# willard-yuan/cvt

Measured on AMD Instinct MI355X. Metric: queries/sec, OPQ-ADC top-100 over 128-d SIFT-1M, higher is better.
Workload: dtype u8 codes / f32 distances

## Files before the change

### cvt_amd/csrc/adc_mfma.hip

```cpp
#include <algorithm>
#include <cfloat>
#include <cmath>

#include "common.h"
#include "flat_f32_common.h"
#include "adc_scan16.h"
#include "kernels.h"
#include "launch.h"

namespace cvtmi {

namespace {

constexpr double MF_UP = 1.0 + 1e-9;
constexpr double MF_BMAX = 4194304.0;
constexpr int MF_NSEL = 4096;
constexpr int MF_KEEP = 512;
constexpr int MF_CALL_WORDS = 64;

__global__ __launch_bounds__(kBlock) void mf_pack_kernel(const uint4 *__restrict__ codes, int64_t n, int ks, int step, const int8_t *__restrict__ xb,
                                                         int64_t tile0, int64_t ntiles, uint4 *__restrict__ pack)
{
    const int64_t g = tile0 * ks * 64 + (int64_t)blockIdx.x * kBlock + threadIdx.x;
    if (g >= ntiles * ks * 64) return;
    const int lane = (int)(g & 63);
    const int64_t ts = g >> 6, t = ts / ks;
    const int s_ = (int)(ts - t * ks);
    const int64_t row = t * 32 + (lane & 31);
    uint32_t w[4] = { 0u, 0u, 0u, 0u };
    if (row < n) {
        const uint4 cv = codes[row];
        const int d0 = 32 * s_ + 16 * (lane >> 5);
#pragma unroll
        for (int e = 0; e < 16; ++e) {
            const int d = d0 + e, m = d / step, kk = d - m * step;
            const uint32_t word = (m >> 2) == 0 ? cv.x : ((m >> 2) == 1 ? cv.y : ((m >> 2) == 2 ? cv.z : cv.w));
            const uint32_t code = (word >> (8 * (m & 3))) & 0xffu;
            w[e >> 2] |= (uint32_t)(uint8_t)xb[((size_t)m * 256 + code) * step + kk] << (8 * (e & 3));
        }
    }
    pack[g] = make_uint4(w[0], w[1], w[2], w[3]);
}

__global__ __launch_bounds__(kBlock) void mf_norm_kernel(const uint4 *__restrict__ codes, int64_t row0, int64_t n, const double *__restrict__ nrm,
                                                         float *__restrict__ norms)
{
    const int64_t row = row0 + (int64_t)blockIdx.x * kBlock + threadIdx.x;
    if (row >= n) return;
    const uint4 cv = codes[row];
    const uint32_t cw[4] = { cv.x, cv.y, cv.z, cv.w };
    double s_ = 0.0;
#pragma unroll
    for (int m = 0; m < 16; ++m) s_ += nrm[m * 256 + ((cw[m >> 2] >> (8 * (m & 3))) & 0xffu)];
    norms[row] = __double2float_ru(s_ * (1.0 + 1e-12));
}

__device__ __forceinline__ double mf_wave_sum(double v)
{
#pragma unroll
    for (int o = 32; o > 0; o >>= 1) v += __shfl_xor(v, o, 64);
    return v;
}

__global__ __launch_bounds__(256) void mf_qmax_kernel(const float *__restrict__ q_rot, const float *__restrict__ centroid, const float *__restrict__ s, int D, int nq,
                                                      uint32_t *__restrict__ wq, uint32_t *__restrict__ flags)
{
    const int q = blockIdx.x * 4 + (threadIdx.x >> 6), lane = threadIdx.x & 63;
    if (q >= nq) return;
    float mx = 0.0f;
    bool fin = true;
    for (int d = lane; d < D; d += 64) {
        const float r = __fsub_rn(q_rot[(int64_t)q * D + d], centroid[d]);
        if (!(fabsf(r) <= FLT_MAX)) fin = false;
        const float w = __double2float_ru(fabs((double)r * (double)s[d]));
        mx = w > mx ? w : mx;
    }
    fin = __ballot(!fin) == 0ull;
    const uint32_t bits = fs_wave_max_u32(__float_as_uint(fin ? mx : 0.0f));
    if (lane == 0) {
        flags[q] = fin ? 0u : 1u;
        wq[q] = bits;
    }
}
__global__ __launch_bounds__(1024) void mf_qred_kernel(const uint32_t *__restrict__ wq, int nq, uint32_t *__restrict__ call)
{
    __shared__ uint32_t part[16];
    uint32_t mx = 0u;
    for (int q = threadIdx.x; q < nq; q += 1024) mx = wq[q] > mx ? wq[q] : mx;
    mx = fs_wave_max_u32(mx);
    if ((threadIdx.x & 63) == 0) part[threadIdx.x >> 6] = mx;
    __syncthreads();
    if (threadIdx.x == 0) {
        for (int w = 1; w < 16; ++w) mx = part[w] > mx ? part[w] : mx;
        call[0] = mx;
    }
}

__device__ __forceinline__ double mf_scale(const uint32_t *call) { return (double)__uint_as_float(call[0]) / 127.0 * (1.0 + 1e-12); }
__device__ __forceinline__ bool mf_scale_ok(double t, double xhat_max) { return t > 0.0 && t <= 1e300 && xhat_max * xhat_max * (1.0 + 1e-6) <= MF_BMAX * 2.0 * t; }

__global__ __launch_bounds__(256) void mf_quant_kernel(const float *__restrict__ q_rot, const float *__restrict__ centroid, const float *__restrict__ s, int D, int nq,
                                                       const uint32_t *__restrict__ call, double x_max, double eps_max, double xhat_max, double gamma,
                                                       int8_t *__restrict__ W, int32_t *__restrict__ margin, uint32_t *__restrict__ flags)
{
    const int q = blockIdx.x * 4 + (threadIdx.x >> 6), lane = threadIdx.x & 63;
    if (q >= nq) return;
    const double t = mf_scale(call);
    const bool usable = mf_scale_ok(t, xhat_max) && flags[q] == 0u;
    double d2 = 0.0, w2 = 0.0, r2 = 0.0;
    for (int d = lane; d < D; d += 64) {
        int Wi = 0;
        if (usable) {
            const double r = (double)__fsub_rn(q_rot[(int64_t)q * D + d], centroid[d]);
            const double w = r * (double)s[d];
            const double u = w / t;
            double Wd = rint(u);
            Wd = Wd > 127.0 ? 127.0 : (Wd < -127.0 ? -127.0 : Wd);
            const double dl = u - Wd;
            Wi = (int)Wd;
            d2 += dl * dl; w2 += w * w; r2 += r * r;
        }
        W[(int64_t)q * D + d] = (int8_t)Wi;
    }
    d2 = mf_wave_sum(d2); w2 = mf_wave_sum(w2); r2 = mf_wave_sum(r2);
    if (lane == 0) {
        const double reach = sqrt(r2) * MF_UP + xhat_max;
        const double fp = gamma * reach * reach + 1e-30;
        const double E = (2.0 * (t * (sqrt(d2) * MF_UP + 1e-9) * x_max + sqrt(w2) * MF_UP * eps_max) + 4.0 * t + fp) * MF_UP;
        const double mg = usable ? ceil(E / t) + 1.0 : 0.0;
        const bool ok = usable && mg < 268435456.0 && reach * reach < 1e37;
        margin[q] = ok ? (int32_t)mg : 0;
        if (!ok) flags[q] = 1u;
    }
}

__global__ __launch_bounds__(kBlock) void mf_bias_kernel(const float *__restrict__ norms, int64_t n, const uint32_t *__restrict__ call, double xhat_max,
                                                         int32_t *__restrict__ bias)
{
    const int64_t row = (int64_t)blockIdx.x * kBlock + threadIdx.x;
    if (row >= n) return;
    const double t = mf_scale(call);
    bias[row] = mf_scale_ok(t, xhat_max) ? (int32_t)floor((double)norms[row] / (2.0 * t)) : 0;
}

template <int NK>
__global__ __launch_bounds__(256) void mf_theta_kernel(const uint32_t *__restrict__ smax, int nq, int k, const int32_t *__restrict__ margin, int32_t *__restrict__ thr,
                                                       uint32_t *__restrict__ cnt, uint32_t *__restrict__ flags)
{
    const int q = blockIdx.x * 4 + (threadIdx.x >> 6), lane = threadIdx.x & 63;
    if (q >= nq) return;
    uint32_t key[NK];
    int present = 0;
#pragma unroll
    for (int j = 0; j < NK; ++j) {
        key[j] = smax[(size_t)q * (NK * 64) + j * 64 + lane];
        present += __popcll(__ballot(key[j] != 0u));
    }
    const uint32_t sel = fs_wave_select(key, k, k + k / 4 + 8);
    if (lane == 0) {
        int32_t th = 0x7fffffff;
        if (flags[q] == 0u) {
            if (sel == 0u || 4 * present < 5 * k) flags[q] = 1u;
            else th = (int32_t)(sel ^ 0x80000000u) - margin[q];
        }
        thr[q] = th;
        cnt[q] = 0u;
    }
}

template <int NK>
__device__ __forceinline__ void mf_select_body(const uint8_t *__restrict__ codes, const float *__restrict__ lut_g, int K, int nq_lut, int64_t q_base, int64_t n, int k,
                                                       const uint32_t *__restrict__ cnt, const uint2 *__restrict__ cand, uint32_t lcap, const int32_t *__restrict__ margin,
                                                       const uint32_t *__restrict__ pass_flag, int64_t id_base, float *__restrict__ out_d,
                                                       int64_t *__restrict__ out_id, uint32_t *__restrict__ flags, unsigned long long *sel, uint32_t nc)
{
    const int lane = threadIdx.x, ql = blockIdx.x;
    const int64_t q = q_base + ql;
    const int64_t want = k < n ? k : n;
    const uint2 *cq = cand + (size_t)ql * lcap;
    uint32_t key[NK];
#pragma unroll
    for (int j = 0; j < NK; ++j) key[j] = (uint32_t)(j * 64 + lane) < nc ? (cq[j * 64 + lane].x ^ 0x80000000u) : 0u;
    const uint32_t a2 = fs_wave_select(key, (int)want, (int)want);
    const uint32_t cut = (uint32_t)((int32_t)(a2 ^ 0x80000000u) - margin[q]) ^ 0x80000000u;
    const ExactFromLut fix{ reinterpret_cast<const uint4 *>(codes), lut_g, K, nq_lut, (int)(q / SQ_QT) };
#pragma unroll
    for (int j = 0; j < NK; ++j) {
        const bool in = key[j] != 0u && key[j] >= cut;
        key[j] = 0u;
        if (__ballot(in) == 0ull) continue;
        if (in) key[j] = ~(uint32_t)(fix((int)(q % SQ_QT), (unsigned long long)cq[j * 64 + lane].y) >> 32);
    }
    const uint32_t kd = fs_wave_select(key, (int)want, (int)want);
    uint32_t ns = 0;
#pragma unroll
    for (int j = 0; j < NK; ++j) {
        const bool in = key[j] != 0u && key[j] >= kd;
        const unsigned long long m = __ballot(in);
        if (m == 0ull) continue;
        const uint32_t pos = ns + __builtin_amdgcn_mbcnt_hi((uint32_t)(m >> 32), __builtin_amdgcn_mbcnt_lo((uint32_t)m, 0u));
        if (in && pos < (uint32_t)MF_KEEP) sel[pos] = ((unsigned long long)(~key[j]) << 32) | cq[j * 64 + lane].y;
        ns += (uint32_t)__popcll(m);
    }
    if (ns > (uint32_t)MF_KEEP) {
        if (lane == 0) flags[q] = 1u;
        return;
    }
    int np = 64;
    while (np < (int)ns) np <<= 1;
    for (int i = (int)ns + lane; i < np; i += 64) sel[i] = ~0ull;
    block_bitonic_u64<64>(sel, np);
    for (int i = lane; i < k; i += 64) {
        if ((uint32_t)i < ns) {
            const unsigned long long e = sel[i];
            out_d[q * k + i] = __uint_as_float((uint32_t)(e >> 32));
            out_id[q * k + i] = id_base + (int64_t)(uint32_t)e;
        } else {
            out_d[q * k + i] = __uint_as_float(0x7f800000u);
            out_id[q * k + i] = -1;
        }
    }
}

__global__ __launch_bounds__(64) void mf_select_kernel(const uint8_t *__restrict__ codes, const float *__restrict__ lut_g, int K, int nq_lut, int64_t q_base, int64_t n, int k,
                                                       const uint32_t *__restrict__ cnt, const uint2 *__restrict__ cand, uint32_t lcap, const int32_t *__restrict__ margin,
                                                       const uint32_t *__restrict__ pass_flag, int qper, int64_t id_base, float *__restrict__ out_d,
                                                       int64_t *__restrict__ out_id, uint32_t *__restrict__ flags)
{
    __shared__ __attribute__((aligned(16))) unsigned long long sel[MF_KEEP];
    const int64_t q = q_base + blockIdx.x;
    const uint32_t nc = cnt[blockIdx.x];
    if (flags[q] != 0u || pass_flag[blockIdx.x / qper] != 0u || nc > lcap || (int64_t)nc < (k < n ? k : n)) {
        if (threadIdx.x == 0) flags[q] = 1u;
        return;
    }
    if (nc <= 1024u) mf_select_body<16>(codes, lut_g, K, nq_lut, q_base, n, k, cnt, cand, lcap, margin, pass_flag, id_base, out_d, out_id, flags, sel, nc);
    else mf_select_body<MF_NSEL / 64>(codes, lut_g, K, nq_lut, q_base, n, k, cnt, cand, lcap, margin, pass_flag, id_base, out_d, out_id, flags, sel, nc);
}

__global__ __launch_bounds__(256) void mf_compact_kernel(const uint32_t *__restrict__ flags, int nq, int D, const float *__restrict__ q_rot, uint32_t *__restrict__ count,
                                                         int cap, int32_t *__restrict__ slot_q, float *__restrict__ q_c, uint32_t *__restrict__ only_c,
                                                         uint32_t *__restrict__ rest)
{
    const int q = blockIdx.x * 4 + (threadIdx.x >> 6), lane = threadIdx.x & 63;
    if (q >= nq) return;
    if (flags[q] == 0u) { if (lane == 0) rest[q] = 0u; return; }
    uint32_t slot = 0;
    if (lane == 0) slot = atomicAdd(count, 1u);
    slot = (uint32_t)__builtin_amdgcn_readfirstlane((int)slot);
    if (slot >= (uint32_t)cap) { if (lane == 0) rest[q] = 1u; return; }
    for (int d = lane; d < D; d += 64) q_c[(size_t)slot * D + d] = q_rot[(int64_t)q * D + d];
    if (lane == 0) { slot_q[slot] = q; only_c[slot] = 1u; rest[q] = 0u; }
}
__global__ __launch_bounds__(128) void mf_scatter_kernel(const int32_t *__restrict__ slot_q, const uint32_t *__restrict__ only_c, int k, const float *__restrict__ d_c,
                                                         const int64_t *__restrict__ i_c, float *__restrict__ dist, int64_t *__restrict__ ids)
{
    const int slot = blockIdx.x;
    if (only_c[slot] == 0u) return;
    const int64_t q = slot_q[slot];
    for (int i = threadIdx.x; i < k; i += 128) { dist[q * k + i] = d_c[(int64_t)slot * k + i]; ids[q * k + i] = i_c[(int64_t)slot * k + i]; }
}

__global__ __launch_bounds__(256) void mf_count_kernel(const uint32_t *__restrict__ flags, int nq, unsigned long long *__restrict__ stat)
{
    const int q = blockIdx.x * 256 + threadIdx.x;
    const unsigned long long m = __ballot(q < nq && flags[q] != 0u);
    if ((threadIdx.x & 63) == 0 && m) atomicAdd(stat + 1, (unsigned long long)__popcll(m));
    if (q == 0) stat[0] = (unsigned long long)nq;
}

size_t mf_align(size_t v, size_t a) { return (v + a - 1) / a * a; }

constexpr size_t MF_PIECE_BYTES = (size_t)1 << 30;
struct MfShape {
    int chunks, qper, spx, stride;
    int64_t regions;
    uint32_t rec_cap;
    size_t bytes;
};
MfShape mf_shape(int D, int64_t n, int64_t m, int k, int list_cap, int div, bool fill = true)
{
    MfShape s;
    s.chunks = (int)blocks_for(m, 256);
    s.qper = (int)(blocks_for(blocks_for(m, s.chunks), 32) * 32);
    s.spx = s.chunks == 1 ? 32 : (s.chunks == 2 ? 16 : 8);
    s.stride = 8 * s.spx * 16;
    s.regions = (int64_t)8 * s.spx * s.chunks * 8;
    const double pass = std::min<double>((double)std::max(4 * k, 256) * div, (double)n);
    const int64_t all_groups = blocks_for(blocks_for(n, 32), u8_filter_rt(D)), streams = (int64_t)8 * s.spx * 8;
    const double share = (double)blocks_for(all_groups, streams) / (double)all_groups;
    const double base = (double)s.qper * pass * share;
    s.rec_cap = (uint32_t)std::min<double>(8192.0, std::max<double>(256.0, 2.0 * base));
    if (fill) {
        const size_t other = mf_align((size_t)m * 4, 256) * 2 + mf_align((size_t)s.chunks * 4, 256) + mf_align((size_t)m * s.stride * 4, 256) +
                             mf_align((size_t)s.regions * 4, 256) + mf_align((size_t)m * list_cap * sizeof(uint2), 256) + 256;
        const size_t room = other < MF_PIECE_BYTES ? (MF_PIECE_BYTES - other) / ((size_t)s.regions * u8_filter_rec_bytes()) : 0;
        const uint32_t want = (uint32_t)std::min<double>(8192.0, 8.0 * base);
        s.rec_cap = std::max(s.rec_cap, (uint32_t)std::min<size_t>(want, room));
    }
    s.bytes = mf_align((size_t)m * 4, 256) * 2 + mf_align((size_t)s.chunks * 4, 256) + mf_align((size_t)m * s.stride * 4, 256) + mf_align((size_t)s.regions * 4, 256) +
              mf_align((size_t)m * list_cap * sizeof(uint2), 256) + mf_align((size_t)s.regions * s.rec_cap * u8_filter_rec_bytes(), 256);
    return s;
}
constexpr int MF_REDO = 64, MF_REDO_SPLITS = 32;
size_t mf_redo_bytes(int D, int k)
{
    return mf_align(MF_REDO * 4, 256) * 2 + mf_align((size_t)MF_REDO * D * 4, 256) + mf_align((size_t)MF_REDO * k * 4, 256) + mf_align((size_t)MF_REDO * k * 8, 256) +
           mf_align((size_t)MF_REDO * MF_REDO_SPLITS * k * 4, 256) + mf_align((size_t)MF_REDO * MF_REDO_SPLITS * k * 8, 256);
}
size_t mf_call_bytes(int D, int64_t n, int64_t nq)
{
    return mf_redo_bytes(D, 128) + mf_align((size_t)nq * 4, 256) + mf_align(MF_CALL_WORDS * 4, 256) + mf_align((size_t)nq * 4, 256) * 2 + mf_align((size_t)nq * D, 256) + mf_align((size_t)n * 4, 256);
}

}

bool adc_mfma_model(const float *books, int D, int K, int8_t *xb, double *nrm, float *c, float *s, double *x_max, double *eps_max, double *xhat_max)
{
    const int M = 16, step = D / M;
    if (K != 256 || D % M != 0) return false;
    for (size_t i = 0; i < (size_t)D * K; ++i)
        if (!std::isfinite(books[i])) return false;
    for (int d = 0; d < D; ++d) {
        const int m = d / step, kk = d % step;
        double lo = books[(size_t)m * K * step + kk], hi = lo;
        for (int j = 1; j < K; ++j) {
            const double v = books[((size_t)m * K + j) * step + kk];
            lo = v < lo ? v : lo; hi = v > hi ? v : hi;
        }
        const double range = hi - lo;
        float cf = (float)(0.5 * hi + 0.5 * lo), sf = (float)(range / 254.0);
        if (range == 0.0) { cf = (float)lo; sf = 0.0f; }
        else if (!(sf >= FLT_MIN) || !std::isfinite(sf) || !std::isfinite(cf)) return false;
        c[d] = cf; s[d] = sf;
    }
    double sx = 0.0, se = 0.0, sn = 0.0;
    for (int m = 0; m < M; ++m) {
        double mx = 0.0, me = 0.0, mn = 0.0;
        for (int j = 0; j < K; ++j) {
            double x2 = 0.0, e2 = 0.0, n2 = 0.0;
            for (int kk = 0; kk < step; ++kk) {
                const int d = m * step + kk;
                const double v = books[((size_t)m * K + j) * step + kk];
                double X = 0.0, e = 0.0;
                if (s[d] > 0.0f) {
                    const double u = (v - (double)c[d]) / (double)s[d];
                    X = std::nearbyint(u);
                    X = X > 127.0 ? 127.0 : (X < -127.0 ? -127.0 : X);
                    e = u - X;
                }
                xb[((size_t)m * 256 + j) * step + kk] = (int8_t)(int)X;
                x2 += X * X; e2 += e * e; n2 += v * v;
            }
            nrm[m * 256 + j] = n2;
            mx = std::max(mx, x2); me = std::max(me, e2); mn = std::max(mn, n2);
        }
        sx += mx; se += me; sn += mn;
    }
    *x_max = std::sqrt(sx) * MF_UP; *eps_max = std::sqrt(se) * MF_UP + 1e-12; *xhat_max = std::sqrt(sn) * MF_UP;
    return std::isfinite(*x_max) && std::isfinite(*eps_max) && std::isfinite(*xhat_max);
}

size_t adc_mfma_pack_bytes(int D, int64_t n) { return (size_t)((n + 31) / 32) * (D / 32) * 64 * sizeof(uint4); }

int launch_adc_mfma_pack(const AdcMfmaModel &mm, int D, const uint8_t *codes, int64_t row0, int64_t n, void *pack, float *norms, hipStream_t st)
{
    if (D % 32 != 0 || D < 32 || D > 256 || row0 < 0 || row0 > n) return fail(CVTMI_EINVAL, "adc_mfma_pack: D=%d rows %lld..%lld", D, (long long)row0, (long long)n);
    if (n == row0) return CVTMI_OK;
    const int ks = D / 32;
    const int64_t ntiles = (n + 31) / 32, tile0 = row0 / 32, total = (ntiles - tile0) * ks * 64;
    CVTMI_TRY(launch("mf_pack_kernel", mf_pack_kernel, blocks_for(total, kBlock), kBlock, 0, st, reinterpret_cast<const uint4 *>(codes), n, ks, D / 16, mm.xb, tile0, ntiles,
                     reinterpret_cast<uint4 *>(pack)));
    return launch("mf_norm_kernel", mf_norm_kernel, blocks_for(n - row0, kBlock), kBlock, 0, st, reinterpret_cast<const uint4 *>(codes), row0, n, mm.nrm, norms);
}

static int mf_div(int sample_div) { return sample_div >= 1 && sample_div <= 3 ? sample_div : 2; }

size_t adc_mfma_scratch_bytes(int D, int64_t n, int64_t nq, int k, int list_cap, int sample_div, int64_t *per)
{
    const int div = mf_div(sample_div);
    int64_t p = nq;
    while (p > 256 && mf_shape(D, n, p, k, list_cap, div, false).bytes > MF_PIECE_BYTES) p = blocks_for(blocks_for(p, 2), 256) * 256;
    if (per) *per = p;
    size_t piece = mf_shape(D, n, p, k, list_cap, div).bytes;
    if (nq % p) piece = std::max(piece, mf_shape(D, n, nq % p, k, list_cap, div).bytes);
    return mf_call_bytes(D, n, nq) + piece;
}

int launch_adc_mfma(const OpqModelDev &m, const AdcMfmaModel &mm, const uint8_t *codes, const void *pack, const float *norms, int64_t n, int64_t id_base,
                    const float *q_rot, int64_t nq, int k, int list_cap, int sample_div, float *lut_g, void *scratch, float *dist, int64_t *ids,
                    AdcMfmaRedo *redo, unsigned long long *stat, hipStream_t st)
{
    if (m.M != 16 || m.K != 256 || m.D % 32 != 0 || m.D > 256 || k < 1 || k > 128 || n < 1 || n >= 0x7fffffe0LL || nq < 1 || nq > 0x7fffffff || list_cap < 1 ||
        list_cap > MF_NSEL)
        return fail(CVTMI_EUNSUPPORTED, "adc_mfma: shape not covered");
    const int D = m.D, div = mf_div(sample_div);
    int64_t per = 0;
    adc_mfma_scratch_bytes(D, n, nq, k, list_cap, sample_div, &per);
    char *sc = reinterpret_cast<char *>(scratch);
    uint32_t *call = reinterpret_cast<uint32_t *>(sc); sc += mf_align(MF_CALL_WORDS * 4, 256);
    uint32_t *flags = reinterpret_cast<uint32_t *>(sc); sc += mf_align((size_t)nq * 4, 256);
    int32_t *margin = reinterpret_cast<int32_t *>(sc); sc += mf_align((size_t)nq * 4, 256);
    int8_t *W = reinterpret_cast<int8_t *>(sc); sc += mf_align((size_t)nq * D, 256);
    int32_t *bias = reinterpret_cast<int32_t *>(sc); sc += mf_align((size_t)n * 4, 256);
    redo->slot_q = reinterpret_cast<int32_t *>(sc); sc += mf_align(MF_REDO * 4, 256);
    redo->only = reinterpret_cast<uint32_t *>(sc); sc += mf_align(MF_REDO * 4, 256);
    redo->q = reinterpret_cast<float *>(sc); sc += mf_align((size_t)MF_REDO * D * 4, 256);
    redo->d = reinterpret_cast<float *>(sc); sc += mf_align((size_t)MF_REDO * 128 * 4, 256);
    redo->i = reinterpret_cast<int64_t *>(sc); sc += mf_align((size_t)MF_REDO * 128 * 8, 256);
    redo->part_d = reinterpret_cast<float *>(sc); sc += mf_align((size_t)MF_REDO * MF_REDO_SPLITS * 128 * 4, 256);
    redo->part_i = reinterpret_cast<int64_t *>(sc); sc += mf_align((size_t)MF_REDO * MF_REDO_SPLITS * 128 * 8, 256);
    redo->rest = reinterpret_cast<uint32_t *>(sc); sc += mf_align((size_t)nq * 4, 256);
    CVTMI_HIP(hipMemsetAsync(call, 0, MF_CALL_WORDS * 4, st));
    const double gamma = (double)(m.step + 24) * 5.9604644775390625e-8 * 1.01;
    CVTMI_TRY(launch_lut(m, q_rot, nq, nullptr, lut_g, st, 256));
    CVTMI_TRY(launch("mf_qmax_kernel", mf_qmax_kernel, blocks_for(nq, 4), 256, 0, st, q_rot, m.coarse, mm.s, D, (int)nq, reinterpret_cast<uint32_t *>(margin), flags));
    CVTMI_TRY(launch("mf_qred_kernel", mf_qred_kernel, 1, 1024, 0, st, reinterpret_cast<const uint32_t *>(margin), (int)nq, call));
    CVTMI_TRY(launch("mf_quant_kernel", mf_quant_kernel, blocks_for(nq, 4), 256, 0, st, q_rot, m.coarse, mm.s, D, (int)nq, call, mm.x_max, mm.eps_max, mm.xhat_max,
                     gamma, W, margin, flags));
    CVTMI_TRY(launch("mf_bias_kernel", mf_bias_kernel, blocks_for(n, kBlock), kBlock, 0, st, norms, n, call, mm.xhat_max, bias));
    const int rt = u8_filter_rt(D);
    const int64_t all_groups = blocks_for(blocks_for(n, 32), rt);
    for (int64_t q0 = 0; q0 < nq; q0 += per) {
        const int64_t mq = std::min(per, nq - q0);
        const MfShape s = mf_shape(D, n, mq, k, list_cap, div);
        char *p = sc;
        int32_t *thr = reinterpret_cast<int32_t *>(p); p += mf_align((size_t)mq * 4, 256);
        uint32_t *cnt = reinterpret_cast<uint32_t *>(p); p += mf_align((size_t)mq * 4, 256);
        uint32_t *cflag = reinterpret_cast<uint32_t *>(p); p += mf_align((size_t)s.chunks * 4, 256);
        uint32_t *smax = reinterpret_cast<uint32_t *>(p); p += mf_align((size_t)mq * s.stride * 4, 256);
        CVTMI_HIP(hipMemsetAsync(cflag, 0, (size_t)s.chunks * 4, st));
        uint32_t *wcnt = reinterpret_cast<uint32_t *>(p); p += mf_align((size_t)s.regions * 4, 256);
        uint2 *cand = reinterpret_cast<uint2 *>(p); p += mf_align((size_t)mq * list_cap * sizeof(uint2), 256);
        void *rec = p;
        U8FilterJob j;
        j.pack = pack; j.bias = bias; j.n = n; j.D = D; j.W = W + q0 * D; j.nq = (int)mq; j.chunks = s.chunks; j.qper = s.qper; j.spx = s.spx;
        j.smax = smax; j.smax_stride = s.stride;
        {
            const int64_t streams = (int64_t)8 * s.spx * 8;
            const int64_t want = std::max<int64_t>(blocks_for(all_groups, div), std::min<int64_t>(all_groups, 2048 / rt));
            j.n_sample = std::min<int64_t>(all_groups, blocks_for(want, streams) * streams);
        }
        j.thr = thr; j.rec = rec; j.wcnt = wcnt; j.rec_cap = s.rec_cap; j.cnt = cnt; j.cand = cand; j.list_cap = (uint32_t)list_cap; j.pass_flag = cflag;
        CVTMI_TRY(launch_u8_filter_sample(j, st));
        auto theta = mf_theta_kernel<16>;
        if (s.stride == 2048) theta = mf_theta_kernel<32>;
        else if (s.stride == 4096) theta = mf_theta_kernel<64>;
        CVTMI_TRY(launch("mf_theta_kernel", theta, blocks_for(mq, 4), 256, 0, st, smax, (int)mq, k, margin + q0, thr, cnt, flags + q0));
        CVTMI_TRY(launch_u8_filter_pass(j, st));
        CVTMI_TRY(launch_u8_filter_bucket(j, st));
        CVTMI_TRY(launch("mf_select_kernel", mf_select_kernel, mq, 64, 0, st, codes, lut_g, m.K, (int)nq, q0, n, k, cnt, cand, (uint32_t)list_cap, margin, cflag, s.qper,
                         id_base, dist, ids, flags));
    }
    if (stat) {
        CVTMI_HIP(hipMemsetAsync(stat, 0, 2 * sizeof(unsigned long long), st));
        CVTMI_TRY(launch("mf_count_kernel", mf_count_kernel, blocks_for(nq, 256), 256, 0, st, flags, (int)nq, stat));
    }
    redo->cap = MF_REDO; redo->splits = n >= (1 << 18) ? MF_REDO_SPLITS : 1;
    CVTMI_HIP(hipMemsetAsync(redo->only, 0, MF_REDO * 4, st));
    CVTMI_HIP(hipMemsetAsync(redo->q, 0, (size_t)MF_REDO * D * 4, st));
    CVTMI_TRY(launch("mf_compact_kernel", mf_compact_kernel, blocks_for(nq, 4), 256, 0, st, flags, (int)nq, D, q_rot, call + MF_CALL_WORDS - 1, MF_REDO, redo->slot_q, redo->q,
                     redo->only, redo->rest));
    return CVTMI_OK;
}

int launch_adc_mfma_scatter(const AdcMfmaRedo &redo, int k, float *dist, int64_t *ids, hipStream_t st)
{
    return launch("mf_scatter_kernel", mf_scatter_kernel, redo.cap, 128, 0, st, redo.slot_q, redo.only, k, redo.d, redo.i, dist, ids);
}

}
```

Measured before the change: 3.738 million.

## Split select kernel by candidate count and batch exact rescoring via LDS band

The select stage becomes two template kernel instantiations, a short form for up to 1024 candidates and a long form launched separately. Each has its own LDS sizing, so short lists no longer carry the register and LDS footprint of the 4096-candidate path. Candidates passing the cut are compacted into an LDS band, then rescored four at a time with a batched exact-LUT helper instead of one divergent per-lane call. Row ids are cached in registers so they are not reloaded from global memory. The risks are an extra kernel launch when list capacity exceeds 1024 and the added syncthreads and band writes.

After: 3.891 million, median of 6. +4.1%, better.

```diff
diff --git a/cvt_amd/csrc/adc_mfma.hip b/cvt_amd/csrc/adc_mfma.hip
--- a/cvt_amd/csrc/adc_mfma.hip
+++ b/cvt_amd/csrc/adc_mfma.hip
@@ -15,6 +15,7 @@
 constexpr double MF_UP = 1.0 + 1e-9;
 constexpr double MF_BMAX = 4194304.0;
 constexpr int MF_NSEL = 4096;
+constexpr int MF_NSHORT = 1024;
 constexpr int MF_KEEP = 512;
 constexpr int MF_CALL_WORDS = 64;
 
@@ -169,28 +170,70 @@
 }
 
 template <int NK>
-__device__ __forceinline__ void mf_select_body(const uint8_t *__restrict__ codes, const float *__restrict__ lut_g, int K, int nq_lut, int64_t q_base, int64_t n, int k,
+__global__ __launch_bounds__(64) void mf_select_kernel(const uint8_t *__restrict__ codes, const float *__restrict__ lut_g, int K, int nq_lut, int64_t q_base, int64_t n, int k,
                                                        const uint32_t *__restrict__ cnt, const uint2 *__restrict__ cand, uint32_t lcap, const int32_t *__restrict__ margin,
-                                                       const uint32_t *__restrict__ pass_flag, int64_t id_base, float *__restrict__ out_d,
-                                                       int64_t *__restrict__ out_id, uint32_t *__restrict__ flags, unsigned long long *sel, uint32_t nc)
-{
+                                                       const uint32_t *__restrict__ pass_flag, int qper, int64_t id_base, float *__restrict__ out_d,
+                                                       int64_t *__restrict__ out_id, uint32_t *__restrict__ flags)
+{
+    __shared__ __attribute__((aligned(16))) unsigned long long sel[NK * 32 > MF_KEEP ? NK * 32 : MF_KEEP];
+    uint32_t *band = reinterpret_cast<uint32_t *>(sel);
     const int lane = threadIdx.x, ql = blockIdx.x;
     const int64_t q = q_base + ql;
     const int64_t want = k < n ? k : n;
+    const uint32_t nc = cnt[ql];
+    static_assert(NK == MF_NSHORT / 64 || NK == MF_NSEL / 64, "the two forms");
+    if constexpr (NK == MF_NSHORT / 64) {
+        if (flags[q] != 0u || pass_flag[ql / qper] != 0u || nc > lcap || (int64_t)nc < want) {
+            if (lane == 0) flags[q] = 1u;
+            return;
+        }
+        if (nc > (uint32_t)MF_NSHORT) return;
+    } else {
+        if (flags[q] != 0u || nc <= (uint32_t)MF_NSHORT) return;
+    }
     const uint2 *cq = cand + (size_t)ql * lcap;
-    uint32_t key[NK];
-#pragma unroll
-    for (int j = 0; j < NK; ++j) key[j] = (uint32_t)(j * 64 + lane) < nc ? (cq[j * 64 + lane].x ^ 0x80000000u) : 0u;
+    uint32_t key[NK], row[NK];
+#pragma unroll
+    for (int j = 0; j < NK; ++j) {
+        const uint32_t i = (uint32_t)(j * 64 + lane);
+        const uint2 e = cq[i < nc ? i : nc - 1u];
+        key[j] = i < nc ? (e.x ^ 0x80000000u) : 0u;
+        row[j] = e.y;
+    }
     const uint32_t a2 = fs_wave_select(key, (int)want, (int)want);
     const uint32_t cut = (uint32_t)((int32_t)(a2 ^ 0x80000000u) - margin[q]) ^ 0x80000000u;
-    const ExactFromLut fix{ reinterpret_cast<const uint4 *>(codes), lut_g, K, nq_lut, (int)(q / SQ_QT) };
+    uint32_t nb = 0;
 #pragma unroll
     for (int j = 0; j < NK; ++j) {
         const bool in = key[j] != 0u && key[j] >= cut;
+        const unsigned long long m = __ballot(in);
+        const uint32_t pos = nb + __builtin_amdgcn_mbcnt_hi((uint32_t)(m >> 32), __builtin_amdgcn_mbcnt_lo((uint32_t)m, 0u));
+        if (in) band[pos] = row[j];
+        nb += (uint32_t)__popcll(m);
         key[j] = 0u;
-        if (__ballot(in) == 0ull) continue;
-        if (in) key[j] = ~(uint32_t)(fix((int)(q % SQ_QT), (unsigned long long)cq[j * 64 + lane].y) >> 32);
-    }
+    }
+    __syncthreads();
+    const ExactFromLutBatch<> fixb{ codes, lut_g, K, nq_lut, (int)(q / SQ_QT) };
+#pragma unroll
+    for (int b = 0; b < NK / 4; ++b) {
+        if ((uint32_t)(b * 256) < nb) {
+            unsigned long long e[4];
+            bool need[4];
+#pragma unroll
+            for (int r = 0; r < 4; ++r) {
+                const uint32_t i = (uint32_t)((4 * b + r) * 64 + lane);
+                need[r] = i < nb;
+                e[r] = band[need[r] ? i : 0u];
+            }
+            fixb((int)(q % SQ_QT), e, need);
+#pragma unroll
+            for (int r = 0; r < 4; ++r) {
+                key[4 * b + r] = need[r] ? ~(uint32_t)(e[r] >> 32) : 0u;
+                row[4 * b + r] = (uint32_t)e[r];
+            }
+        }
+    }
+    __syncthreads();
     const uint32_t kd = fs_wave_select(key, (int)want, (int)want);
     uint32_t ns = 0;
 #pragma unroll
@@ -199,7 +242,7 @@
         const unsigned long long m = __ballot(in);
         if (m == 0ull) continue;
         const uint32_t pos = ns + __builtin_amdgcn_mbcnt_hi((uint32_t)(m >> 32), __builtin_amdgcn_mbcnt_lo((uint32_t)m, 0u));
-        if (in && pos < (uint32_t)MF_KEEP) sel[pos] = ((unsigned long long)(~key[j]) << 32) | cq[j * 64 + lane].y;
+        if (in && pos < (uint32_t)MF_KEEP) sel[pos] = ((unsigned long long)(~key[j]) << 32) | row[j];
         ns += (uint32_t)__popcll(m);
     }
     if (ns > (uint32_t)MF_KEEP) {
@@ -220,22 +263,6 @@
             out_id[q * k + i] = -1;
         }
     }
-}
-
-__global__ __launch_bounds__(64) void mf_select_kernel(const uint8_t *__restrict__ codes, const float *__restrict__ lut_g, int K, int nq_lut, int64_t q_base, int64_t n, int k,
-                                                       const uint32_t *__restrict__ cnt, const uint2 *__restrict__ cand, uint32_t lcap, const int32_t *__restrict__ margin,
-                                                       const uint32_t *__restrict__ pass_flag, int qper, int64_t id_base, float *__restrict__ out_d,
-                                                       int64_t *__restrict__ out_id, uint32_t *__restrict__ flags)
-{
-    __shared__ __attribute__((aligned(16))) unsigned long long sel[MF_KEEP];
-    const int64_t q = q_base + blockIdx.x;
-    const uint32_t nc = cnt[blockIdx.x];
-    if (flags[q] != 0u || pass_flag[blockIdx.x / qper] != 0u || nc > lcap || (int64_t)nc < (k < n ? k : n)) {
-        if (threadIdx.x == 0) flags[q] = 1u;
-        return;
-    }
-    if (nc <= 1024u) mf_select_body<16>(codes, lut_g, K, nq_lut, q_base, n, k, cnt, cand, lcap, margin, pass_flag, id_base, out_d, out_id, flags, sel, nc);
-    else mf_select_body<MF_NSEL / 64>(codes, lut_g, K, nq_lut, q_base, n, k, cnt, cand, lcap, margin, pass_flag, id_base, out_d, out_id, flags, sel, nc);
 }
 
 __global__ __launch_bounds__(256) void mf_compact_kernel(const uint32_t *__restrict__ flags, int nq, int D, const float *__restrict__ q_rot, uint32_t *__restrict__ count,
@@ -449,8 +476,11 @@
         CVTMI_TRY(launch("mf_theta_kernel", theta, blocks_for(mq, 4), 256, 0, st, smax, (int)mq, k, margin + q0, thr, cnt, flags + q0));
         CVTMI_TRY(launch_u8_filter_pass(j, st));
         CVTMI_TRY(launch_u8_filter_bucket(j, st));
-        CVTMI_TRY(launch("mf_select_kernel", mf_select_kernel, mq, 64, 0, st, codes, lut_g, m.K, (int)nq, q0, n, k, cnt, cand, (uint32_t)list_cap, margin, cflag, s.qper,
+        CVTMI_TRY(launch("mf_select_kernel", mf_select_kernel<MF_NSHORT / 64>, mq, 64, 0, st, codes, lut_g, m.K, (int)nq, q0, n, k, cnt, cand, (uint32_t)list_cap, margin, cflag, s.qper,
                          id_base, dist, ids, flags));
+        if (list_cap > MF_NSHORT)
+            CVTMI_TRY(launch("mf_select_long_kernel", mf_select_kernel<MF_NSEL / 64>, mq, 64, 0, st, codes, lut_g, m.K, (int)nq, q0, n, k, cnt, cand, (uint32_t)list_cap, margin,
+                             cflag, s.qper, id_base, dist, ids, flags));
     }
     if (stat) {
         CVTMI_HIP(hipMemsetAsync(stat, 0, 2 * sizeof(unsigned long long), st));
```
